# isarandi/metrabs

Measured on AMD Instinct MI355X. Metric: crops/sec (256px, 72 depth bins) at 1/2/4/8 MI355X; MPJPE vs ref, higher is better.
Workload: dtype f32

## Files before the change

metrabs_amd/build.py:

```python
import hashlib
import os
import shutil
import subprocess
import sys
from concurrent.futures import ThreadPoolExecutor

CSRC = os.path.join(os.path.dirname(os.path.abspath(__file__)), 'csrc')
LIB_PATH = os.path.join(CSRC, 'libmetrabs_hip.so')
BUILD_DIR = os.path.join(CSRC, 'build')
ARCH = 'gfx950'
FLAGS = ['-O3', '-std=c++17', '-fPIC', f'--offload-arch={ARCH}', '-Wall', '-Wno-unused-function',
         '-Wno-inline-asm']
EXTRA_FLAGS = {'head_rt.hip': ['-mllvm', '-amdgpu-mfma-vgpr-form=1'],
               'depthwise5x5.hip': ['-fno-slp-vectorize']}


def sources():
    return sorted(f for f in os.listdir(CSRC) if f.endswith('.hip'))


def _hipcc():
    exe = shutil.which('hipcc') or '/opt/rocm/bin/hipcc'
    if not os.path.exists(exe):
        raise RuntimeError('hipcc not found; metrabs_amd needs ROCm to build its HIP kernels')
    return exe


def _digest(path):
    h = hashlib.sha256()
    h.update(' '.join(FLAGS + EXTRA_FLAGS.get(os.path.basename(path), [])).encode())
    for dep in [path] + [os.path.join(CSRC, f) for f in sorted(os.listdir(CSRC)) if f.endswith('.h')] \
            + [os.path.join(os.path.dirname(os.path.dirname(CSRC)), 'include', 'metrabs_hip.h')]:
        with open(dep, 'rb') as f:
            h.update(f.read())
    return h.hexdigest()


def _compile(src, force):
    path = os.path.join(CSRC, src)
    obj = os.path.join(BUILD_DIR, src + '.o')
    stamp = obj + '.sha256'
    digest = _digest(path)
    if not force and os.path.exists(obj) and os.path.exists(stamp) and open(stamp).read() == digest:
        return obj, False
    cmd = [_hipcc(), *FLAGS, *EXTRA_FLAGS.get(src, []), '-c', path, '-o', obj]
    r = subprocess.run(cmd, capture_output=True, text=True)
    if r.returncode != 0:
        raise RuntimeError(f'hipcc failed for {src}:\n{r.stdout}\n{r.stderr}')
    if r.stderr.strip():
        sys.stderr.write(r.stderr)
    with open(stamp, 'w') as f:
        f.write(digest)
    return obj, True


def build_library(force=False, verbose=True):
    os.makedirs(BUILD_DIR, exist_ok=True)
    srcs = sources()
    with ThreadPoolExecutor(max_workers=min(8, len(srcs))) as ex:
        results = list(ex.map(lambda s: _compile(s, force), srcs))
    objs = [o for o, _ in results]
    rebuilt = any(r for _, r in results)
    if rebuilt or force or not os.path.exists(LIB_PATH):
        cmd = [_hipcc(), '-shared', '-fPIC', f'--offload-arch={ARCH}', *objs, '-o', LIB_PATH]
        r = subprocess.run(cmd, capture_output=True, text=True)
        if r.returncode != 0:
            raise RuntimeError(f'link failed:\n{r.stdout}\n{r.stderr}')
        if verbose:
            print(f'built {LIB_PATH} from {len(srcs)} sources')
    elif verbose:
        print(f'{LIB_PATH} is up to date')
    return LIB_PATH


def kernel_resources(src):
    import re
    import tempfile
    path = os.path.join(CSRC, src)
    with tempfile.TemporaryDirectory() as tmp:
        asm = os.path.join(tmp, src + '.s')
        cmd = [_hipcc(), *[f for f in FLAGS if f != '-fPIC'], *EXTRA_FLAGS.get(src, []), '-S',
               '--cuda-device-only', path, '-o', asm]
        r = subprocess.run(cmd, capture_output=True, text=True)
        if r.returncode != 0:
            raise RuntimeError(f'hipcc -S failed for {src}:\n{r.stderr}')
        text = open(asm).read()
    loops = mfma_loop_lane_traffic(text)
    out = []
    meta = text[text.index('amdhsa.kernels:'):] if 'amdhsa.kernels:' in text else ''
    for blk in re.split(r'\n  - ', meta)[1:]:
        if '.vgpr_count:' not in blk:
            continue
        get = lambda k: int(re.search(rf'\.{k}:\s+(\d+)', blk).group(1))
        name = re.search(r'\.name:\s+(\S+)', blk).group(1)
        out.append(dict(name=name, mfma_loops=loops.get(name, []),
                        **{k: get(k) for k in ('vgpr_count', 'agpr_count', 'vgpr_spill_count',
                                               'sgpr_spill_count', 'private_segment_fixed_size',
                                               'group_segment_fixed_size')}))
    return out


def mfma_loop_lane_traffic(asm_text):
    import re
    out = {}
    for m in re.finditer(r'^(_Z\w+):[^\n]*\n', asm_text, flags=re.M):
        name = m.group(1)
        end = asm_text.find('.Lfunc_end', m.end())
        if end < 0:
            continue
        body = asm_text[m.end():end].split('\n')
        labels = {}
        for i, line in enumerate(body):
            lm = re.match(r'^(\.LBB\d+_\d+):', line)
            if lm:
                labels[lm.group(1)] = i
        spans = []
        for i, line in enumerate(body):
            bm = re.search(r's_c?branch\S*\s+(\.LBB\d+_\d+)', line)
            if bm and labels.get(bm.group(1), 1 << 30) <= i:
                spans.append((labels[bm.group(1)], i))
        inner = [sp for sp in spans if not any(o != sp and sp[0] <= o[0] and o[1] <= sp[1] for o in spans)]
        loops = []
        for a, b in inner:
            seg = body[a:b + 1]
            n = lambda key: sum(key in x for x in seg)
            if n('v_mfma'):
                loops.append(dict(mfma=n('v_mfma'), lane_moves=n('v_readlane') + n('v_writelane'),
                                  barriers=n('s_barrier'), dma=n('global_load_lds')))
        out[name] = loops
    return out


if __name__ == '__main__':
    build_library(force='--force' in sys.argv)
```

metrabs_amd/csrc/conv1x1.hip:

```cpp
#include <type_traits>

#include "common.h"

namespace mtr {

typedef float f32x16 __attribute__((ext_vector_type(16)));

constexpr int kC1PadX = 32;
constexpr int kC1PadW = 4;

template <int WM, int WN, int FM, int FN, int BK, int ACT, int PRE>
__global__ __launch_bounds__(64 * WM * WN) void conv1x1_kernel(
    const float* __restrict__ x, const float* __restrict__ w, const float* __restrict__ bias,
    const float* __restrict__ in_bias, const float* __restrict__ gate, const float* __restrict__ residual,
    float* __restrict__ y, int M, int K, int HW, int n_total, FastDiv by_hw) {
  constexpr int NT = 64 * WM * WN;
  constexpr int BM = 32 * FM * WM, BN = 32 * FN * WN;
  constexpr int LDX = BN + kC1PadX, LDW = BM + kC1PadW;
  constexpr int XROW4 = BN / 4;
  constexpr int XPASS = NT / XROW4;
  constexpr int XV = (BK + XPASS - 1) / XPASS;
  constexpr int WPASS = NT / (BK / 4);
  constexpr int WV = (BM + WPASS - 1) / WPASS;
  static_assert(NT % XROW4 == 0 && NT % (BK / 4) == 0, "loader mapping");
  __shared__ float xs[2][BK * LDX];
  __shared__ float ws[2][BK * LDW];

  const int tid = threadIdx.x, lane = tid & 63, wave = tid >> 6;
  const int wm = wave % WM, wn = wave / WM;
  const int m0 = blockIdx.y * BM, n0 = blockIdx.x * BN;
  const long long khw = (long long)K * HW;

  const int xn4 = tid % XROW4, xk0 = tid / XROW4;
  const int xcol = n0 + xn4 * 4;
  const bool xcol_ok = xcol < n_total;
  const unsigned xb = xcol_ok ? fastdiv((unsigned)xcol, by_hw) : 0u;
  const float* xsrc = x + (long long)xb * khw + (xcol - (int)xb * HW);
  const float* gsrc = gate ? gate + (long long)xb * K : nullptr;
  const int wk4 = tid % (BK / 4), wr0 = tid / (BK / 4);

  float4 xr[XV], wr[WV];
  auto load_tile = [&](int k0) {
#pragma unroll
    for (int v = 0; v < XV; ++v) {
      const int k = k0 + xk0 + v * XPASS;
      float4 t = make_float4(0.0f, 0.0f, 0.0f, 0.0f);
      if (xcol_ok && k < K && xk0 + v * XPASS < BK) {
        t = *reinterpret_cast<const float4*>(xsrc + (long long)k * HW);
        if constexpr (PRE >= 0) {
          const float bi = in_bias[k];
          t.x = settled(activate<PRE>(t.x + bi)); t.y = settled(activate<PRE>(t.y + bi));
          t.z = settled(activate<PRE>(t.z + bi)); t.w = settled(activate<PRE>(t.w + bi));
        }
        if (gsrc) {
          const float g = gsrc[k];
          t.x *= g; t.y *= g; t.z *= g; t.w *= g;
        }
      }
      xr[v] = t;
    }
#pragma unroll
    for (int v = 0; v < WV; ++v) {
      const int m = m0 + wr0 + v * WPASS, k = k0 + wk4 * 4;
      float4 t = make_float4(0.0f, 0.0f, 0.0f, 0.0f);
      if (m < M && k < K && wr0 + v * WPASS < BM) t = *reinterpret_cast<const float4*>(w + (long long)m * K + k);
      wr[v] = t;
    }
  };
  auto store_tile = [&](int buf) {
#pragma unroll
    for (int v = 0; v < XV; ++v) {
      const int r = xk0 + v * XPASS;
      if (r < BK) *reinterpret_cast<float4*>(&xs[buf][r * LDX + xn4 * 4]) = xr[v];
    }
#pragma unroll
    for (int v = 0; v < WV; ++v) {
      const int r = wr0 + v * WPASS;
      if (r < BM) {
        float* d = &ws[buf][(wk4 * 4) * LDW + r];
        d[0] = wr[v].x; d[LDW] = wr[v].y; d[2 * LDW] = wr[v].z; d[3 * LDW] = wr[v].w;
      }
    }
  };

  f32x16 acc[FM][FN];
#pragma unroll
  for (int i = 0; i < FM; ++i)
#pragma unroll
    for (int j = 0; j < FN; ++j)
#pragma unroll
      for (int r = 0; r < 16; ++r) acc[i][j][r] = 0.0f;

  const int half = lane >> 5, l32 = lane & 31;
  const int n_tiles = (K + BK - 1) / BK;
  load_tile(0);
  store_tile(0);
  __syncthreads();
  for (int t = 0; t < n_tiles; ++t) {
    const int buf = t & 1;
    if (t + 1 < n_tiles) load_tile((t + 1) * BK);
    const float* xb_ = &xs[buf][half * LDX + wn * (32 * FN) + l32];
    const float* wb_ = &ws[buf][half * LDW + wm * (32 * FM) + l32];
#pragma unroll
    for (int kk = 0; kk < BK; kk += 2) {
      float a[FN], b[FM];
#pragma unroll
      for (int j = 0; j < FN; ++j) a[j] = xb_[kk * LDX + j * 32];
#pragma unroll
      for (int i = 0; i < FM; ++i) b[i] = wb_[kk * LDW + i * 32];
#pragma unroll
      for (int i = 0; i < FM; ++i)
#pragma unroll
        for (int j = 0; j < FN; ++j) acc[i][j] = __builtin_amdgcn_mfma_f32_32x32x2f32(a[j], b[i], acc[i][j], 0, 0, 0);
    }
    if (t + 1 < n_tiles) store_tile(buf ^ 1);
    __syncthreads();
  }

#pragma unroll
  for (int i = 0; i < FM; ++i) {
    const int m = m0 + wm * (32 * FM) + i * 32 + l32;
    if (m >= M) continue;
    const float bm = bias[m];
#pragma unroll
    for (int j = 0; j < FN; ++j) {
#pragma unroll
      for (int g = 0; g < 4; ++g) {
        const int col = n0 + wn * (32 * FN) + j * 32 + 8 * g + 4 * half;
        if (col >= n_total) continue;
        const unsigned b = fastdiv((unsigned)col, by_hw);
        const long long off = ((long long)b * M + m) * HW + (col - (int)b * HW);
        float4 r;
        r.x = activate<ACT>(acc[i][j][4 * g + 0] + bm);
        r.y = activate<ACT>(acc[i][j][4 * g + 1] + bm);
        r.z = activate<ACT>(acc[i][j][4 * g + 2] + bm);
        r.w = activate<ACT>(acc[i][j][4 * g + 3] + bm);
        if (residual) {
          const float4 q = *reinterpret_cast<const float4*>(residual + off);
          r.x += q.x; r.y += q.y; r.z += q.z; r.w += q.w;
        }
        *reinterpret_cast<float4*>(y + off) = r;
      }
    }
  }
}

constexpr int kDkBK = 32, kDkBN = 16, kDkStages = 3;
constexpr int kDkLDW = kDkBK + 4;

typedef float f32x4 __attribute__((ext_vector_type(4)));

constexpr size_t deepk_lds_bytes(int waves) {
  return (size_t)kDkStages * (kDkBK * kDkBN + 32 * waves * kDkLDW) * sizeof(float);
}

template <int WAVES, int ACT, int PRE>
__global__ __launch_bounds__(64 * WAVES) void conv1x1_deepk_kernel(
    const float* __restrict__ x, const float* __restrict__ w, const float* __restrict__ bias,
    const float* __restrict__ in_bias, const float* __restrict__ gate, const float* __restrict__ residual,
    float* __restrict__ y, int M, int K, int HW, int n_total, FastDiv by_hw) {
  constexpr int NT = 64 * WAVES, BM = 32 * WAVES;
  constexpr int XS = kDkBK * kDkBN, WS = BM * kDkLDW;
  static_assert(BM * (kDkBK / 4) == 4 * NT, "W loader mapping");
  extern __shared__ float4 dk_lds[];
  float* xs = reinterpret_cast<float*>(dk_lds);
  float* ws = xs + kDkStages * XS;

  const int tid = threadIdx.x, lane = tid & 63, wave = tid >> 6;
  const int m0 = blockIdx.y * BM, n0 = blockIdx.x * kDkBN;
  const long long khw = (long long)K * HW;

  constexpr int XV = XS / NT;
  static_assert(XV * NT == XS && (XV == 1 || XV == 2), "x loader mapping");
  const int xp = (tid % (kDkBN / XV)) * XV, xk = tid / (kDkBN / XV);
  const int xcol = n0 + xp;
  const bool xcol_ok = xcol < n_total;
  const unsigned xb = xcol_ok ? fastdiv((unsigned)xcol, by_hw) : 0u;
  const float* xsrc = xcol_ok ? x + (long long)xb * khw + (xcol - (int)xb * HW) : x;
  const bool has_gate = gate != nullptr;
  const float* gsrc = has_gate ? gate + (long long)xb * K : x;
  const int wk4 = tid & 7, wr0 = tid >> 3;

  const float4 zero = make_float4(0.0f, 0.0f, 0.0f, 0.0f);
  float4 rw[2][4] = {{zero, zero, zero, zero}, {zero, zero, zero, zero}};
  float rx[2][XV] = {}, rg[2] = {1.0f, 1.0f}, rbi[2] = {0.0f, 0.0f};
  auto load_tile = [&](int kt, auto set) {
    constexpr int P = decltype(set)::value;
    const int k0 = kt * kDkBK;
    const int kx = min(k0 + xk, K - 1);
    if constexpr (XV == 2) {
      const float2 t = *reinterpret_cast<const float2*>(xsrc + (long long)kx * HW);
      rx[P][0] = t.x; rx[P][XV - 1] = t.y;
    } else {
      rx[P][0] = xsrc[(long long)kx * HW];
    }
    rg[P] = gsrc[kx];
    if constexpr (PRE >= 0) rbi[P] = in_bias[kx];
    const int k = min(k0 + wk4 * 4, K - 4);
#pragma unroll
    for (int v = 0; v < 4; ++v) {
      const int m = min(m0 + wr0 + v * (NT / 8), M - 1);
      rw[P][v] = *reinterpret_cast<const float4*>(w + (long long)m * K + k);
    }
  };
  auto store_tile = [&](int stage, int kt, auto set) {
    constexpr int P = decltype(set)::value;
    const int k0 = kt * kDkBK;
    const float g = has_gate ? rg[P] : 1.0f;
    const bool x_ok = xcol_ok && k0 + xk < K;
    float* xd = &xs[stage * XS + xk * kDkBN + xp];
    float v0 = rx[P][0], v1 = rx[P][XV - 1];
    if constexpr (PRE >= 0) {
      v0 = settled(activate<PRE>(v0 + rbi[P]));
      if constexpr (XV == 2) v1 = settled(activate<PRE>(v1 + rbi[P]));
    }
    if constexpr (XV == 2) {
      *reinterpret_cast<float2*>(xd) = make_float2(x_ok ? v0 * g : 0.0f, x_ok ? v1 * g : 0.0f);
    } else {
      *xd = x_ok ? v0 * g : 0.0f;
    }
    const bool k_ok = k0 + wk4 * 4 < K;
#pragma unroll
    for (int v = 0; v < 4; ++v) {
      const int row = wr0 + v * (NT / 8);
      const bool ok = k_ok && m0 + row < M;
      float4 u = rw[P][v];
      u.x = ok ? u.x : 0.0f; u.y = ok ? u.y : 0.0f; u.z = ok ? u.z : 0.0f; u.w = ok ? u.w : 0.0f;
      *reinterpret_cast<float4*>(&ws[stage * WS + row * kDkLDW + wk4 * 4]) = u;
    }
  };

  f32x4 acc[2];
#pragma unroll
  for (int f = 0; f < 2; ++f)
#pragma unroll
    for (int r = 0; r < 4; ++r) acc[f][r] = 0.0f;

  const int c = lane & 15, kg = lane >> 4;
  auto multiply = [&](int stage, int kk0) {
    const float* xb_ = &xs[stage * XS + kg * kDkBN + c];
    const float* wb_ = &ws[stage * WS + (wave * 32 + c) * kDkLDW + kg];
#pragma unroll
    for (int kk = kk0; kk < kk0 + kDkBK / 2; kk += 4) {
      const float a = xb_[kk * kDkBN];
      const float b0 = wb_[kk], b1 = wb_[16 * kDkLDW + kk];
      acc[0] = __builtin_amdgcn_mfma_f32_16x16x4f32(a, b0, acc[0], 0, 0, 0);
      acc[1] = __builtin_amdgcn_mfma_f32_16x16x4f32(a, b1, acc[1], 0, 0, 0);
    }
  };

  const int n_tiles = (K + kDkBK - 1) / kDkBK;
  constexpr std::integral_constant<int, 0> ra{};
  constexpr std::integral_constant<int, 1> rb{};
  load_tile(0, ra);
  if (n_tiles > 1) load_tile(1, rb);
  store_tile(0, 0, ra);
  if (n_tiles > 1) store_tile(1, 1, rb);
  if (n_tiles > 2) load_tile(2, ra);
  __syncthreads();
  int stage = 0;
  auto step = [&](int t, auto hold, auto issue, auto guarded) {
    constexpr bool G = decltype(guarded)::value;
    if (!G || t + 3 < n_tiles) load_tile(t + 3, issue);
    multiply(stage, 0);
    __builtin_amdgcn_sched_barrier(0);
    if (!G || t + 2 < n_tiles) store_tile(stage == 0 ? 2 : stage - 1, t + 2, hold);
    __builtin_amdgcn_sched_barrier(0);
    multiply(stage, kDkBK / 2);
    stage = stage == 2 ? 0 : stage + 1;
    __syncthreads();
  };
  int t = 0;
  for (; t + 4 < n_tiles; t += 2) {
    step(t, ra, rb, std::false_type{});
    step(t + 1, rb, ra, std::false_type{});
  }
  for (; t < n_tiles; t += 2) {
    step(t, ra, rb, std::true_type{});
    if (t + 1 < n_tiles) step(t + 1, rb, ra, std::true_type{});
  }

  const int col = n0 + 4 * kg;
  if (col >= n_total) return;
  const unsigned b = fastdiv((unsigned)col, by_hw);
#pragma unroll
  for (int f = 0; f < 2; ++f) {
    const int m = m0 + wave * 32 + f * 16 + c;
    if (m >= M) continue;
    const float bm = bias[m];
    const long long off = ((long long)b * M + m) * HW + (col - (int)b * HW);
    float4 r;
    r.x = activate<ACT>(acc[f][0] + bm);
    r.y = activate<ACT>(acc[f][1] + bm);
    r.z = activate<ACT>(acc[f][2] + bm);
    r.w = activate<ACT>(acc[f][3] + bm);
    if (residual) {
      const float4 q = *reinterpret_cast<const float4*>(residual + off);
      r.x += q.x; r.y += q.y; r.z += q.z; r.w += q.w;
    }
    *reinterpret_cast<float4*>(y + off) = r;
  }
}

constexpr int kD6BM = 64, kD6BN = 64, kD6BK = 32, kD6Stages = 3, kD6Waves = 8;
constexpr int kD6LDW = kD6BK + 2;

template <int ACT, int PRE>
__global__ __launch_bounds__(64 * kD6Waves) void conv1x1_deep64_kernel(
    const float* __restrict__ x, const float* __restrict__ w, const float* __restrict__ bias,
    const float* __restrict__ in_bias, const float* __restrict__ gate, const float* __restrict__ residual,
    float* __restrict__ y, int M, int K, int HW, int n_total, FastDiv by_hw) {
  constexpr int NT = 64 * kD6Waves, BM = kD6BM, BN = kD6BN, BK = kD6BK, LDW = kD6LDW;
  constexpr int XS = BK * BN, WS = BM * LDW;
  static_assert(BK * (BN / 4) == NT && BM * (BK / 4) == NT, "loader mappings: one 16-byte group of x and of W each");
  __shared__ __attribute__((aligned(16))) float d6_lds[kD6Stages * (XS + WS)];
  float* xs = d6_lds;
  float* ws = d6_lds + kD6Stages * XS;

  const int tid = threadIdx.x, lane = tid & 63, wave = tid >> 6;
  const int wm = wave & 1, wn = wave >> 1;
  const int m0 = blockIdx.y * BM, n0 = blockIdx.x * BN;
  const long long khw = (long long)K * HW;

  const int xn4 = tid & 15, xk = tid >> 4;
  const int xcol = n0 + 4 * xn4;
  const bool xcol_ok = xcol < n_total;
  const unsigned xb = xcol_ok ? fastdiv((unsigned)xcol, by_hw) : 0u;
  const float* xsrc = xcol_ok ? x + (long long)xb * khw + (xcol - (int)xb * HW) : x;
  const bool has_gate = gate != nullptr;
  const float* gsrc = has_gate ? gate + (long long)xb * K : x;
  const int xdst = xk * BN + ((4 * xn4) ^ ((xk & 1) << 4));
  const int wk4 = tid & 7, wr = tid >> 3;
  const float* wsrc = w + (long long)min(m0 + wr, M - 1) * K;
  const bool wrow_ok = m0 + wr < M;
  const int wdst = wr * LDW + 4 * wk4;
  const float* xcur = xsrc + (long long)(3 * BK + xk) * HW;
  const float* gcur = gsrc + 3 * BK + xk;
  const float* bcur = PRE >= 0 ? in_bias + 3 * BK + xk : nullptr;
  const float* wcur = wsrc + 3 * BK + 4 * wk4;
  const long long xadv = (long long)BK * HW;

  const float4 zero = make_float4(0.0f, 0.0f, 0.0f, 0.0f);
  float4 rx[2] = {zero, zero}, rw[2] = {zero, zero};
  float rg[2] = {1.0f, 1.0f}, rbi[2] = {0.0f, 0.0f};
  auto load_tile = [&](int kt, auto set) {
    constexpr int P = decltype(set)::value;
    const int k0 = kt * BK;
    const int kx = min(k0 + xk, K - 1);
    rx[P] = *reinterpret_cast<const float4*>(xsrc + (long long)kx * HW);
    rg[P] = gsrc[kx];
    if constexpr (PRE >= 0) rbi[P] = in_bias[kx];
    rw[P] = *reinterpret_cast<const float4*>(wsrc + min(k0 + 4 * wk4, K - 4));
  };
  auto load_next_whole_tile = [&](auto set) {
    constexpr int P = decltype(set)::value;
    rx[P] = *reinterpret_cast<const float4*>(xcur);
    rg[P] = *gcur;
    if constexpr (PRE >= 0) rbi[P] = *bcur;
    rw[P] = *reinterpret_cast<const float4*>(wcur);
    xcur += xadv; gcur += BK; wcur += BK;
    if constexpr (PRE >= 0) bcur += BK;
  };
  auto store_tile = [&](int stage, int kt, auto set) {
    constexpr int P = decltype(set)::value;
    const int k0 = kt * BK;
    const float g = has_gate ? rg[P] : 1.0f;
    const bool x_ok = xcol_ok && k0 + xk < K;
    float4 v = rx[P];
    if constexpr (PRE >= 0) {
      const float bi = rbi[P];
      v.x = settled(activate<PRE>(v.x + bi)); v.y = settled(activate<PRE>(v.y + bi));
      v.z = settled(activate<PRE>(v.z + bi)); v.w = settled(activate<PRE>(v.w + bi));
    }
    v.x = x_ok ? v.x * g : 0.0f; v.y = x_ok ? v.y * g : 0.0f; v.z = x_ok ? v.z * g : 0.0f; v.w = x_ok ? v.w * g : 0.0f;
    *reinterpret_cast<float4*>(&xs[stage * XS + xdst]) = v;
    const bool ok = wrow_ok && k0 + 4 * wk4 < K;
    const float4 u = rw[P];
    float* wd = &ws[stage * WS + wdst];
    *reinterpret_cast<float2*>(wd) = make_float2(ok ? u.x : 0.0f, ok ? u.y : 0.0f);
    *reinterpret_cast<float2*>(wd + 2) = make_float2(ok ? u.z : 0.0f, ok ? u.w : 0.0f);
  };

  f32x4 acc[2];
#pragma unroll
  for (int f = 0; f < 2; ++f)
#pragma unroll
    for (int r = 0; r < 4; ++r) acc[f][r] = 0.0f;

  const int c = lane & 15, kg = lane >> 4;
  const int xfrag = kg * BN + ((wn * 16 + c) ^ ((kg & 1) << 4));
  const int wfrag = (wm * 32 + c) * LDW + kg;
  auto multiply = [&](int stage, int kk0) {
    const float* xb_ = &xs[stage * XS + xfrag];
    const float* wb_ = &ws[stage * WS + wfrag];
#pragma unroll
    for (int kk = kk0; kk < kk0 + BK / 2; kk += 4) {
      const float a = xb_[kk * BN];
      const float b0 = wb_[kk], b1 = wb_[16 * LDW + kk];
      acc[0] = __builtin_amdgcn_mfma_f32_16x16x4f32(a, b0, acc[0], 0, 0, 0);
      acc[1] = __builtin_amdgcn_mfma_f32_16x16x4f32(a, b1, acc[1], 0, 0, 0);
    }
  };

  const int n_tiles = (K + BK - 1) / BK, n_whole = K / BK;
  constexpr std::integral_constant<int, 0> ra{};
  constexpr std::integral_constant<int, 1> rb{};
  load_tile(0, ra);
  if (n_tiles > 1) load_tile(1, rb);
  store_tile(0, 0, ra);
  if (n_tiles > 1) store_tile(1, 1, rb);
  if (n_tiles > 2) load_tile(2, ra);
  __syncthreads();
  int stage = 0;
  auto step = [&](int t, auto hold, auto issue, auto guarded) {
    constexpr bool G = decltype(guarded)::value;
    if constexpr (!G) load_next_whole_tile(issue);
    else if (t + 3 < n_tiles) load_tile(t + 3, issue);
    multiply(stage, 0);
    __builtin_amdgcn_sched_barrier(0);
    if (!G || t + 2 < n_tiles) store_tile(stage == 0 ? 2 : stage - 1, t + 2, hold);
    __builtin_amdgcn_sched_barrier(0);
    multiply(stage, BK / 2);
    stage = stage == 2 ? 0 : stage + 1;
    __syncthreads();
  };
  int t = 0;
  for (; t + 4 < n_whole; t += 2) {
    step(t, ra, rb, std::false_type{});
    step(t + 1, rb, ra, std::false_type{});
  }
  for (; t < n_tiles; t += 2) {
    step(t, ra, rb, std::true_type{});
    if (t + 1 < n_tiles) step(t + 1, rb, ra, std::true_type{});
  }

  const int col = n0 + wn * 16 + 4 * kg;
  if (col >= n_total) return;
  const unsigned b = fastdiv((unsigned)col, by_hw);
#pragma unroll
  for (int f = 0; f < 2; ++f) {
    const int m = m0 + wm * 32 + f * 16 + c;
    if (m >= M) continue;
    const float bm = bias[m];
    const long long off = ((long long)b * M + m) * HW + (col - (int)b * HW);
    float4 r;
    r.x = activate<ACT>(acc[f][0] + bm);
    r.y = activate<ACT>(acc[f][1] + bm);
    r.z = activate<ACT>(acc[f][2] + bm);
    r.w = activate<ACT>(acc[f][3] + bm);
    if (residual) {
      const float4 q = *reinterpret_cast<const float4*>(residual + off);
      r.x += q.x; r.y += q.y; r.z += q.z; r.w += q.w;
    }
    *reinterpret_cast<float4*>(y + off) = r;
  }
}

constexpr int kStR = 16;
constexpr int kStWaves = 4;
constexpr size_t kStMaxWeight = 64 * 1024;

inline int stream_kpad(int K) { return (K + 2 * kStR - 1) / (2 * kStR) * (2 * kStR); }
inline bool stream_fits(int M, int K) {
  return M <= 96 && (size_t)stream_kpad(K) * ((M + 31) / 32 * 32) * sizeof(float) <= kStMaxWeight;
}

template <int MT, int PRE, bool GATE>
__global__ __launch_bounds__(64 * kStWaves) void conv1x1_stream_kernel(
    const float* __restrict__ x, const float* __restrict__ w, const float* __restrict__ bias,
    const float* __restrict__ in_bias, const float* __restrict__ gate, const float* __restrict__ residual,
    float* __restrict__ y, int M, int K, int HW, int n_total, FastDiv by_hw, int act, int tiles) {
  constexpr int NT = 64 * kStWaves, LDW = 32 * MT;
  extern __shared__ float4 st_lds[];
  const int Kpad = (K + 2 * kStR - 1) / (2 * kStR) * (2 * kStR);
  float* ws = reinterpret_cast<float*>(st_lds);
  float* bs = ws + Kpad * LDW;

  const int tid = threadIdx.x, lane = tid & 63, wave = tid >> 6;
  const int half = lane >> 5, l32 = lane & 31;
  const long long khw = (long long)K * HW;
  const int n_chunks = Kpad / (2 * kStR);
  const int n0 = blockIdx.x * (32 * kStWaves * tiles);

  int col0 = 0;
  bool ok = false;
  const float* xsrc = x;
  const float* gsrc = x;
  auto enter_tile = [&](int tile) {
    col0 = n0 + tile * 32;
    const int col = col0 + l32;
    ok = col < n_total;
    const unsigned b = ok ? fastdiv((unsigned)col, by_hw) : 0u;
    xsrc = x + (long long)b * khw + (long long)half * HW + (ok ? col - (int)b * HW : 0);
    if constexpr (GATE) gsrc = gate + (long long)b * K + half;
  };

  float xa[kStR], xb[kStR], ga[kStR], gb[kStR];
  auto load_chunk = [&](int c, float (&xr)[kStR], float (&gr)[kStR]) {
#pragma unroll
    for (int j = 0; j < kStR; ++j) {
      const int kk = min(c * (2 * kStR) + 2 * j, K - 2);
      xr[j] = xsrc[(long long)kk * HW];
      if constexpr (GATE) gr[j] = gsrc[kk];
    }
  };

  f32x16 acc[MT];
  auto multiply_chunk = [&](int c, const float (&xr)[kStR], const float (&gr)[kStR]) {
#pragma unroll
    for (int j = 0; j < kStR; ++j) {
      const int k = c * (2 * kStR) + 2 * j;
      float v = xr[j];
      if constexpr (PRE >= 0) v = settled(activate<PRE>(v + bs[k + half]));
      if constexpr (GATE) v *= gr[j];
      v = (ok && k < K) ? v : 0.0f;
      const float* wb_ = &ws[(k + half) * LDW + l32];
#pragma unroll
      for (int i = 0; i < MT; ++i) acc[i] = __builtin_amdgcn_mfma_f32_32x32x2f32(v, wb_[i * 32], acc[i], 0, 0, 0);
    }
  };

  enter_tile(wave);
  load_chunk(0, xa, ga);

  for (int e = tid; e < (Kpad / 4) * LDW; e += NT) {
    const int m = e % LDW, k = (e / LDW) * 4;
    float4 t = make_float4(0.0f, 0.0f, 0.0f, 0.0f);
    if (m < M && k < K) t = *reinterpret_cast<const float4*>(w + (long long)m * K + k);
    float* d = &ws[k * LDW + m];
    d[0] = t.x; d[LDW] = t.y; d[2 * LDW] = t.z; d[3 * LDW] = t.w;
  }
  if constexpr (PRE >= 0)
    for (int k = tid; k < Kpad; k += NT) bs[k] = k < K ? in_bias[k] : 0.0f;
  __syncthreads();

  for (int tile = wave;;) {
#pragma unroll
    for (int i = 0; i < MT; ++i)
#pragma unroll
      for (int r = 0; r < 16; ++r) acc[i][r] = 0.0f;
    int c = 0;
    for (; c + 1 < n_chunks; c += 2) {
      load_chunk(c + 1, xb, gb);
      multiply_chunk(c, xa, ga);
      load_chunk(c + 2, xa, ga);
      multiply_chunk(c + 1, xb, gb);
    }
    if (c < n_chunks) multiply_chunk(c, xa, ga);

    auto epilogue = [&](auto act_c) {
      constexpr int ACT = decltype(act_c)::value;
#pragma unroll
      for (int i = 0; i < MT; ++i) {
        const int m = i * 32 + l32;
        if (m >= M) continue;
        const float bm = bias[m];
#pragma unroll
        for (int g = 0; g < 4; ++g) {
          const int col = col0 + 8 * g + 4 * half;
          if (col >= n_total) continue;
          const unsigned b = fastdiv((unsigned)col, by_hw);
          const long long off = ((long long)b * M + m) * HW + (col - (int)b * HW);
          float4 r;
          r.x = activate<ACT>(acc[i][4 * g + 0] + bm);
          r.y = activate<ACT>(acc[i][4 * g + 1] + bm);
          r.z = activate<ACT>(acc[i][4 * g + 2] + bm);
          r.w = activate<ACT>(acc[i][4 * g + 3] + bm);
          if (residual) {
            const float4 q = *reinterpret_cast<const float4*>(residual + off);
            r.x += q.x; r.y += q.y; r.z += q.z; r.w += q.w;
          }
          *reinterpret_cast<float4*>(y + off) = r;
        }
      }
    };
    switch (act) {
      case kActRelu: epilogue(std::integral_constant<int, kActRelu>{}); break;
      case kActSilu: epilogue(std::integral_constant<int, kActSilu>{}); break;
      case kActHardswish: epilogue(std::integral_constant<int, kActHardswish>{}); break;
      default: epilogue(std::integral_constant<int, kActNone>{}); break;
    }

    tile += kStWaves;
    if (tile >= kStWaves * tiles) break;
    enter_tile(tile);
    load_chunk(0, xa, ga);
  }
}

enum Conv1x1Config {
  kCfgWide = 0, kCfgSquare = 1, kCfgTall = 2, kCfgDeepK = 3, kCfgStream = 4, kCfgDeep64 = 5, kCfgCount = 6
};

struct Conv1x1Plan { int cfg, waves_m, bm, bn; };

inline Conv1x1Plan plan_tall(int M) {
  const int w = M <= 160 ? (M + 31) / 32 : 4;
  return {kCfgTall, w, 32 * w, 32};
}
inline Conv1x1Plan plan_deepk(int M) {
  const int w = M <= 128 ? 4 : 8;
  return {kCfgDeepK, w, 32 * w, kDkBN};
}

inline Conv1x1Plan plan_deep64() { return {kCfgDeep64, 2, kD6BM, kD6BN}; }

inline Conv1x1Plan plan_stream(int M, int K, int HW, long long B) {
  if (!stream_fits(M, K)) return plan_tall(M);
  const int t = (B * HW + 127) / 128 >= 2048 ? 2 : 1;
  return {kCfgStream, (M + 31) / 32, (M + 31) / 32 * 32, 32 * kStWaves * t};
}

inline bool deep64_measured_faster(int M, int K, int HW) {
  static const int classes[][3] = {
      {256, 64, 1024}, {128, 256, 256}, {512, 128, 256}, {128, 512, 256},
      {160, 768, 256}, {960, 160, 256}, {160, 960, 256},
      {256, 960, 64},  {1536, 256, 64}, {256, 1536, 64}, {1280, 256, 64},
  };
  for (const auto& c : classes)
    if (c[0] == M && c[1] == K && c[2] == HW) return true;
  return false;
}

inline Conv1x1Plan pick_config(int M, int K, int HW, long long B) {
  const long long n_total = B * HW;
  const long long n_tiles128 = (n_total + 127) / 128;
  if (deep64_measured_faster(M, K, HW)) return plan_deep64();
  if (M == 48 && K <= 192 && HW == 4096 && stream_fits(M, K)) return plan_stream(M, K, HW, B);
  if (M <= 160) return plan_tall(M);
  if (M == 256 && K >= 512) return HW <= 64 ? plan_deepk(M) : plan_tall(M);
  if (M >= 1024 && M % 128 == 0 && K <= 256 && n_tiles128 <= 32) return plan_tall(M);
  if (M % 192 == 0 && (M / 192) * n_tiles128 >= 512) return {kCfgWide, 2, 192, 128};
  return {kCfgSquare, 2, 128, 128};
}

inline int plan_for(int M, int K, int HW, long long B, int config, Conv1x1Plan* p) {
  switch (config) {
    case -1: *p = pick_config(M, K, HW, B); return MTR_OK;
    case kCfgWide: *p = {kCfgWide, 2, 192, 128}; return MTR_OK;
    case kCfgSquare: *p = {kCfgSquare, 2, 128, 128}; return MTR_OK;
    case kCfgTall: *p = plan_tall(M); return MTR_OK;
    case kCfgDeepK: *p = plan_deepk(M); return MTR_OK;
    case kCfgStream: *p = plan_stream(M, K, HW, B); return MTR_OK;
    case kCfgDeep64: *p = plan_deep64(); return MTR_OK;
    default: return MTR_E_PARAM;
  }
}

template <int WM, int WN, int FM, int FN, int BK, int PRE>
static int launch_conv1x1_pre(const float* x, const float* w, const float* bias, const float* in_bias,
                              const float* gate, const float* residual, float* y, int act, int M, int K, int HW,
                              long long n_total, hipStream_t stream) {
  constexpr int BM = 32 * FM * WM, BN = 32 * FN * WN;
  const long long gx = (n_total + BN - 1) / BN, gy = (M + BM - 1) / BM;
  if (gx > 0x7fffffffLL || gy > 65535) return MTR_E_SHAPE;
  const dim3 grid((unsigned)gx, (unsigned)gy), block(64 * WM * WN);
  const FastDiv by_hw = make_fastdiv((unsigned)HW);
  MTR_CLEAR_STALE();
#define MTR_C1_LAUNCH(ACT)                                                                                      \
  hipLaunchKernelGGL((conv1x1_kernel<WM, WN, FM, FN, BK, ACT, PRE>), grid, block, 0, stream, x, w, bias, in_bias, \
                     gate, residual, y, M, K, HW, (int)n_total, by_hw)
  switch (act) {
    case kActNone: MTR_C1_LAUNCH(kActNone); break;
    case kActRelu: MTR_C1_LAUNCH(kActRelu); break;
    case kActSilu: MTR_C1_LAUNCH(kActSilu); break;
    case kActHardswish: MTR_C1_LAUNCH(kActHardswish); break;
    default: return MTR_E_PARAM;
  }
#undef MTR_C1_LAUNCH
  MTR_CHECK_LAUNCH();
  return MTR_OK;
}

template <int WM, int WN, int FM, int FN, int BK>
static int launch_conv1x1_cfg(const float* x, const float* w, const float* bias, const float* in_bias, int in_act,
                              const float* gate, const float* residual, float* y, int act, int M, int K, int HW,
                              long long n_total, hipStream_t stream) {
#define MTR_C1_PRE(PRE) \
  launch_conv1x1_pre<WM, WN, FM, FN, BK, PRE>(x, w, bias, in_bias, gate, residual, y, act, M, K, HW, n_total, stream)
  switch (in_bias ? in_act : -1) {
    case -1: return MTR_C1_PRE(-1);
    case kActNone: return MTR_C1_PRE(kActNone);
    case kActRelu: return MTR_C1_PRE(kActRelu);
    case kActSilu: return MTR_C1_PRE(kActSilu);
    case kActHardswish: return MTR_C1_PRE(kActHardswish);
    default: return MTR_E_PARAM;
  }
#undef MTR_C1_PRE
}

template <int WAVES, int PRE>
static int launch_conv1x1_deepk_pre(const float* x, const float* w, const float* bias, const float* in_bias,
                                    const float* gate, const float* residual, float* y, int act, int M, int K,
                                    int HW, long long n_total, hipStream_t stream) {
  constexpr int BM = 32 * WAVES;
  constexpr size_t lds = deepk_lds_bytes(WAVES);
  const long long gx = (n_total + kDkBN - 1) / kDkBN, gy = (M + BM - 1) / BM;
  if (gx > 0x7fffffffLL || gy > 65535) return MTR_E_SHAPE;
  const dim3 grid((unsigned)gx, (unsigned)gy), block(64 * WAVES);
  const FastDiv by_hw = make_fastdiv((unsigned)HW);
#define MTR_DK_LAUNCH(ACT)                                                                                 \
  do {                                                                                                     \
    if (lds > 64 * 1024) {                                                                                 \
      const int e = allow_dynamic_lds((const void*)conv1x1_deepk_kernel<WAVES, ACT, PRE>, lds);            \
      if (e != MTR_OK) return e;                                                                           \
    }                                                                                                      \
    MTR_CLEAR_STALE();                                                                                     \
    hipLaunchKernelGGL((conv1x1_deepk_kernel<WAVES, ACT, PRE>), grid, block, lds, stream, x, w, bias,      \
                       in_bias, gate, residual, y, M, K, HW, (int)n_total, by_hw);                         \
  } while (0)
  switch (act) {
    case kActNone: MTR_DK_LAUNCH(kActNone); break;
    case kActRelu: MTR_DK_LAUNCH(kActRelu); break;
    case kActSilu: MTR_DK_LAUNCH(kActSilu); break;
    case kActHardswish: MTR_DK_LAUNCH(kActHardswish); break;
    default: return MTR_E_PARAM;
  }
#undef MTR_DK_LAUNCH
  MTR_CHECK_LAUNCH();
  return MTR_OK;
}

template <int WAVES>
static int launch_conv1x1_deepk(const float* x, const float* w, const float* bias, const float* in_bias,
                                int in_act, const float* gate, const float* residual, float* y, int act, int M,
                                int K, int HW, long long n_total, hipStream_t stream) {
#define MTR_DK_PRE(PRE) \
  launch_conv1x1_deepk_pre<WAVES, PRE>(x, w, bias, in_bias, gate, residual, y, act, M, K, HW, n_total, stream)
  switch (in_bias ? in_act : -1) {
    case -1: return MTR_DK_PRE(-1);
    case kActNone: return MTR_DK_PRE(kActNone);
    case kActRelu: return MTR_DK_PRE(kActRelu);
    case kActSilu: return MTR_DK_PRE(kActSilu);
    case kActHardswish: return MTR_DK_PRE(kActHardswish);
    default: return MTR_E_PARAM;
  }
#undef MTR_DK_PRE
}

template <int PRE>
static int launch_conv1x1_deep64_pre(const float* x, const float* w, const float* bias, const float* in_bias,
                                     const float* gate, const float* residual, float* y, int act, int M, int K,
                                     int HW, long long n_total, hipStream_t stream) {
  const long long gx = (n_total + kD6BN - 1) / kD6BN, gy = (M + kD6BM - 1) / kD6BM;
  if (gx > 0x7fffffffLL || gy > 65535) return MTR_E_SHAPE;
  const dim3 grid((unsigned)gx, (unsigned)gy), block(64 * kD6Waves);
  const FastDiv by_hw = make_fastdiv((unsigned)HW);
  MTR_CLEAR_STALE();
#define MTR_D6_LAUNCH(ACT)                                                                                    \
  hipLaunchKernelGGL((conv1x1_deep64_kernel<ACT, PRE>), grid, block, 0, stream, x, w, bias, in_bias, gate,    \
                     residual, y, M, K, HW, (int)n_total, by_hw)
  switch (act) {
    case kActNone: MTR_D6_LAUNCH(kActNone); break;
    case kActRelu: MTR_D6_LAUNCH(kActRelu); break;
    case kActSilu: MTR_D6_LAUNCH(kActSilu); break;
    case kActHardswish: MTR_D6_LAUNCH(kActHardswish); break;
    default: return MTR_E_PARAM;
  }
#undef MTR_D6_LAUNCH
  MTR_CHECK_LAUNCH();
  return MTR_OK;
}

static int launch_conv1x1_deep64(const float* x, const float* w, const float* bias, const float* in_bias,
                                 int in_act, const float* gate, const float* residual, float* y, int act, int M,
                                 int K, int HW, long long n_total, hipStream_t stream) {
#define MTR_D6_PRE(PRE) \
  launch_conv1x1_deep64_pre<PRE>(x, w, bias, in_bias, gate, residual, y, act, M, K, HW, n_total, stream)
  switch (in_bias ? in_act : -1) {
    case -1: return MTR_D6_PRE(-1);
    case kActNone: return MTR_D6_PRE(kActNone);
    case kActRelu: return MTR_D6_PRE(kActRelu);
    case kActSilu: return MTR_D6_PRE(kActSilu);
    case kActHardswish: return MTR_D6_PRE(kActHardswish);
    default: return MTR_E_PARAM;
  }
#undef MTR_D6_PRE
}

template <int MT, int PRE>
static int launch_conv1x1_stream_pre(const float* x, const float* w, const float* bias, const float* in_bias,
                                     const float* gate, const float* residual, float* y, int act, int M, int K,
                                     int HW, long long n_total, int bn, hipStream_t stream) {
  const int kpad = stream_kpad(K);
  const size_t lds = ((size_t)kpad * 32 * MT + (PRE >= 0 ? kpad : 0)) * sizeof(float);
  const long long gx = (n_total + bn - 1) / bn;
  if (gx > 0x7fffffffLL) return MTR_E_SHAPE;
  if (act < kActNone || act > kActHardswish) return MTR_E_PARAM;
  const dim3 grid((unsigned)gx), block(64 * kStWaves);
  const FastDiv by_hw = make_fastdiv((unsigned)HW);
#define MTR_ST_LAUNCH(GATE)                                                                               \
  do {                                                                                                    \
    if (lds > 64 * 1024) {                                                                                \
      const int e = allow_dynamic_lds((const void*)conv1x1_stream_kernel<MT, PRE, GATE>, lds);            \
      if (e != MTR_OK) return e;                                                                          \
    }                                                                                                     \
    MTR_CLEAR_STALE();                                                                                    \
    hipLaunchKernelGGL((conv1x1_stream_kernel<MT, PRE, GATE>), grid, block, lds, stream, x, w, bias,      \
                       in_bias, gate, residual, y, M, K, HW, (int)n_total, by_hw, act,                    \
                       bn / (32 * kStWaves));                                                             \
  } while (0)
  if (gate) MTR_ST_LAUNCH(true); else MTR_ST_LAUNCH(false);
#undef MTR_ST_LAUNCH
  MTR_CHECK_LAUNCH();
  return MTR_OK;
}

template <int MT>
static int launch_conv1x1_stream(const float* x, const float* w, const float* bias, const float* in_bias,
                                 int in_act, const float* gate, const float* residual, float* y, int act, int M,
                                 int K, int HW, long long n_total, int bn, hipStream_t stream) {
#define MTR_ST_PRE(PRE) \
  launch_conv1x1_stream_pre<MT, PRE>(x, w, bias, in_bias, gate, residual, y, act, M, K, HW, n_total, bn, stream)
  switch (in_bias ? in_act : -1) {
    case -1: return MTR_ST_PRE(-1);
    case kActNone: return MTR_ST_PRE(kActNone);
    case kActRelu: return MTR_ST_PRE(kActRelu);
    case kActSilu: return MTR_ST_PRE(kActSilu);
    case kActHardswish: return MTR_ST_PRE(kActHardswish);
    default: return MTR_E_PARAM;
  }
#undef MTR_ST_PRE
}

}

extern "C" int mtr_conv1x1_plan(int M, int K, int HW, long long B, int config, int* plan) {
  if (!plan) return MTR_E_NULL;
  if (B < 0 || M <= 0 || K <= 0 || HW <= 0) return MTR_E_SHAPE;
  mtr::Conv1x1Plan p;
  const int e = mtr::plan_for(M, K, HW, B, config, &p);
  if (e != MTR_OK) return e;
  plan[0] = p.cfg; plan[1] = p.waves_m; plan[2] = p.bm; plan[3] = p.bn;
  return MTR_OK;
}

extern "C" int mtr_conv1x1_bias_act(const void* x, int dtype, const float* weight, const float* bias,
                                    const float* gate, const void* residual, int act, long long B, int M,
                                    int K, int HW, void* y, mtr_stream_t stream) {
  return mtr_conv1x1_bias_act_pre(x, dtype, weight, bias, nullptr, mtr::kActNone, gate, residual, act, B, M, K, HW, y,
                                  stream, -1);
}

extern "C" int mtr_conv1x1_bias_act_opts(const void* x, int dtype, const float* weight, const float* bias,
                                         const float* gate, const void* residual, int act, long long B,
                                         int M, int K, int HW, void* y, mtr_stream_t stream, int config) {
  if (config > mtr::kCfgDeepK) return x && weight && bias && y ? MTR_E_PARAM : MTR_E_NULL;
  return mtr_conv1x1_bias_act_pre(x, dtype, weight, bias, nullptr, mtr::kActNone, gate, residual, act, B, M, K, HW, y,
                                  stream, config);
}

extern "C" int mtr_conv1x1_bias_act_pre(const void* x, int dtype, const float* weight, const float* bias,
                                        const float* in_bias, int in_act, const float* gate, const void* residual,
                                        int act, long long B, int M, int K, int HW, void* y, mtr_stream_t stream,
                                        int config) {
  if (!x || !weight || !bias || !y) return MTR_E_NULL;
  if (dtype != MTR_F32) return MTR_E_DTYPE;
  if (B < 0 || M <= 0 || K <= 0 || HW <= 0) return MTR_E_SHAPE;
  if (HW % 4 || K % 4) return MTR_E_SHAPE;
  if (B * HW > 0x7fffffffLL || (long long)K * HW > 0x7fffffffLL || (long long)M * HW > 0x7fffffffLL)
    return MTR_E_SHAPE;
  if (act < mtr::kActNone || act > mtr::kActHardswish) return MTR_E_PARAM;
  if (in_act < mtr::kActNone || in_act > mtr::kActHardswish) return MTR_E_PARAM;
  if (!in_bias && in_act != mtr::kActNone) return MTR_E_PARAM;
  if (((uintptr_t)x % 16) || ((uintptr_t)weight % 16) || ((uintptr_t)y % 16) || ((uintptr_t)residual % 16) ||
      ((uintptr_t)in_bias % 4))
    return MTR_E_ALIGN;
  if (x == y || (residual && residual == x)) return MTR_E_PARAM;
  if (B == 0) return MTR_OK;
  const float* xf = (const float*)x;
  const float* rf = (const float*)residual;
  float* yf = (float*)y;
  const long long n_total = B * HW;
  hipStream_t s = (hipStream_t)stream;
  mtr::Conv1x1Plan p;
  if (mtr::plan_for(M, K, HW, B, config, &p) != MTR_OK) return MTR_E_PARAM;
#define MTR_C1_ARGS xf, weight, bias, in_bias, in_act, gate, rf, yf, act, M, K, HW, n_total, s
#define MTR_C1_ARGS_ST xf, weight, bias, in_bias, in_act, gate, rf, yf, act, M, K, HW, n_total, p.bn, s
  switch (p.cfg) {
    case mtr::kCfgWide: return mtr::launch_conv1x1_cfg<2, 2, 3, 2, 16>(MTR_C1_ARGS);
    case mtr::kCfgSquare: return mtr::launch_conv1x1_cfg<2, 2, 2, 2, 16>(MTR_C1_ARGS);
    case mtr::kCfgStream:
      switch (p.waves_m) {
        case 1: return mtr::launch_conv1x1_stream<1>(MTR_C1_ARGS_ST);
        case 2: return mtr::launch_conv1x1_stream<2>(MTR_C1_ARGS_ST);
        default: return mtr::launch_conv1x1_stream<3>(MTR_C1_ARGS_ST);
      }
    case mtr::kCfgDeep64: return mtr::launch_conv1x1_deep64(MTR_C1_ARGS);
    case mtr::kCfgDeepK:
      switch (p.waves_m) {
        case 4: return mtr::launch_conv1x1_deepk<4>(MTR_C1_ARGS);
        default: return mtr::launch_conv1x1_deepk<8>(MTR_C1_ARGS);
      }
    default:
      switch (p.waves_m) {
        case 1: return mtr::launch_conv1x1_cfg<1, 1, 1, 1, 16>(MTR_C1_ARGS);
        case 2: return mtr::launch_conv1x1_cfg<2, 1, 1, 1, 16>(MTR_C1_ARGS);
        case 3: return mtr::launch_conv1x1_cfg<3, 1, 1, 1, 16>(MTR_C1_ARGS);
        case 4: return mtr::launch_conv1x1_cfg<4, 1, 1, 1, 32>(MTR_C1_ARGS);
        default: return mtr::launch_conv1x1_cfg<5, 1, 1, 1, 16>(MTR_C1_ARGS);
      }
  }
#undef MTR_C1_ARGS
#undef MTR_C1_ARGS_ST
}
```

Measured before the change: 9400.

## Restructure streaming conv1x1: per-wave column tiles, float2 loads, smaller chunks, tight LDS

Reworks the streaming 1x1 conv kernel so each wave owns one 32- or 64-column tile instead of looping over several tiles, and adds an NW=2 variant that loads two adjacent columns per lane with float2 and reuses each LDS weight fetch across two MFMA accumulator sets. The chunk depth drops from 16 to 4 k-pairs to cut register pressure, and a tail-free fast loop uses pointer increments plus sched_barriers to keep loads and MFMAs interleaved. LDS weight stride now pads M to 16 instead of 32*MT, and launch bounds request higher occupancy for small tiles. The build script also reports load/MFMA runs and vmcnt waits for inspection. Risks include launch-config mismatch (bn must be 128 or 256) and fewer columns per block amortising the weight LDS fill.

```diff
diff --git a/metrabs_amd/build.py b/metrabs_amd/build.py
--- a/metrabs_amd/build.py
+++ b/metrabs_amd/build.py
@@ -125,8 +125,17 @@
             seg = body[a:b + 1]
             n = lambda key: sum(key in x for x in seg)
             if n('v_mfma'):
+                runs = []
+                for x in seg:
+                    kind = 'M' if 'v_mfma' in x else 'L' if re.match(r'\s*(global|buffer|flat)_load_', x) else None
+                    if kind and runs and runs[-1][0] == kind:
+                        runs[-1][1] += 1
+                    elif kind:
+                        runs.append([kind, 1])
+                waits = [int(v) for x in seg if 's_waitcnt' in x for v in re.findall(r'vmcnt\((\d+)\)', x)]
                 loops.append(dict(mfma=n('v_mfma'), lane_moves=n('v_readlane') + n('v_writelane'),
-                                  barriers=n('s_barrier'), dma=n('global_load_lds')))
+                                  barriers=n('s_barrier'), dma=n('global_load_lds'),
+                                  load_mfma_runs=runs, vmcnt_waits=waits))
         out[name] = loops
     return out
 
diff --git a/metrabs_amd/csrc/conv1x1.hip b/metrabs_amd/csrc/conv1x1.hip
--- a/metrabs_amd/csrc/conv1x1.hip
+++ b/metrabs_amd/csrc/conv1x1.hip
@@ -457,6 +457,7 @@
 }
 
 constexpr int kStR = 16;
+constexpr int kStC = 4;
 constexpr int kStWaves = 4;
 constexpr size_t kStMaxWeight = 64 * 1024;
 
@@ -464,63 +465,90 @@
 inline bool stream_fits(int M, int K) {
   return M <= 96 && (size_t)stream_kpad(K) * ((M + 31) / 32 * 32) * sizeof(float) <= kStMaxWeight;
 }
-
-template <int MT, int PRE, bool GATE>
-__global__ __launch_bounds__(64 * kStWaves) void conv1x1_stream_kernel(
+inline __host__ __device__ int stream_ldw(int M) { return (M + 15) / 16 * 16; }
+constexpr int kStTailPad = 16;
+
+template <int MT, int PRE, bool GATE, int NW>
+__global__ __launch_bounds__(64 * kStWaves, (MT * NW <= 4 && !GATE) ? 4 : 1) void conv1x1_stream_kernel(
     const float* __restrict__ x, const float* __restrict__ w, const float* __restrict__ bias,
     const float* __restrict__ in_bias, const float* __restrict__ gate, const float* __restrict__ residual,
-    float* __restrict__ y, int M, int K, int HW, int n_total, FastDiv by_hw, int act, int tiles) {
-  constexpr int NT = 64 * kStWaves, LDW = 32 * MT;
+    float* __restrict__ y, int M, int K, int HW, int n_total, FastDiv by_hw, int act) {
+  constexpr int NT = 64 * kStWaves, CK = 2 * kStC;
+  const int LDW = stream_ldw(M);
+  static_assert(NW == 1 || NW == 2, "one 4-byte or one 8-byte load per lane and k-step");
   extern __shared__ float4 st_lds[];
   const int Kpad = (K + 2 * kStR - 1) / (2 * kStR) * (2 * kStR);
   float* ws = reinterpret_cast<float*>(st_lds);
-  float* bs = ws + Kpad * LDW;
+  float* bs = ws + Kpad * LDW + kStTailPad;
 
   const int tid = threadIdx.x, lane = tid & 63, wave = tid >> 6;
   const int half = lane >> 5, l32 = lane & 31;
   const long long khw = (long long)K * HW;
-  const int n_chunks = Kpad / (2 * kStR);
-  const int n0 = blockIdx.x * (32 * kStWaves * tiles);
-
-  int col0 = 0;
-  bool ok = false;
-  const float* xsrc = x;
-  const float* gsrc = x;
-  auto enter_tile = [&](int tile) {
-    col0 = n0 + tile * 32;
-    const int col = col0 + l32;
-    ok = col < n_total;
-    const unsigned b = ok ? fastdiv((unsigned)col, by_hw) : 0u;
-    xsrc = x + (long long)b * khw + (long long)half * HW + (ok ? col - (int)b * HW : 0);
-    if constexpr (GATE) gsrc = gate + (long long)b * K + half;
-  };
-
-  float xa[kStR], xb[kStR], ga[kStR], gb[kStR];
-  auto load_chunk = [&](int c, float (&xr)[kStR], float (&gr)[kStR]) {
-#pragma unroll
-    for (int j = 0; j < kStR; ++j) {
-      const int kk = min(c * (2 * kStR) + 2 * j, K - 2);
-      xr[j] = xsrc[(long long)kk * HW];
+  const int n_chunks = Kpad / CK, n_whole = K / CK;
+
+  const int col0 = (blockIdx.x * kStWaves + wave) * (32 * NW);
+  const int lcol = col0 + NW * l32;
+  const bool ok = lcol < n_total;
+  const unsigned lb = ok ? fastdiv((unsigned)lcol, by_hw) : 0u;
+  const float* xsrc = x + (long long)lb * khw + (long long)half * HW + (ok ? lcol - (int)lb * HW : 0);
+  const float* gsrc = GATE ? gate + (long long)lb * K + half : x;
+  const float* xcur = xsrc + (long long)CK * HW;
+  const float* gcur = gsrc + CK;
+  const long long xadv = (long long)CK * HW;
+
+  float xa[kStC][NW], xb[kStC][NW], ga[kStC], gb[kStC];
+  auto load_at = [&](const float* p, float (&d)[NW]) {
+    if constexpr (NW == 2) {
+      const float2 t = *reinterpret_cast<const float2*>(p);
+      d[0] = t.x; d[1] = t.y;
+    } else {
+      d[0] = *p;
+    }
+  };
+  auto load_chunk = [&](int c, float (&xr)[kStC][NW], float (&gr)[kStC]) {
+#pragma unroll
+    for (int j = 0; j < kStC; ++j) {
+      const int kk = min(c * CK + 2 * j, K - 2);
+      load_at(xsrc + (long long)kk * HW, xr[j]);
       if constexpr (GATE) gr[j] = gsrc[kk];
     }
   };
-
-  f32x16 acc[MT];
-  auto multiply_chunk = [&](int c, const float (&xr)[kStR], const float (&gr)[kStR]) {
-#pragma unroll
-    for (int j = 0; j < kStR; ++j) {
-      const int k = c * (2 * kStR) + 2 * j;
-      float v = xr[j];
-      if constexpr (PRE >= 0) v = settled(activate<PRE>(v + bs[k + half]));
-      if constexpr (GATE) v *= gr[j];
-      v = (ok && k < K) ? v : 0.0f;
+  auto load_next_whole_chunk = [&](float (&xr)[kStC][NW], float (&gr)[kStC]) {
+#pragma unroll
+    for (int j = 0; j < kStC; ++j) {
+      load_at(xcur + (long long)(2 * j) * HW, xr[j]);
+      if constexpr (GATE) gr[j] = gcur[2 * j];
+    }
+    xcur += xadv;
+    if constexpr (GATE) gcur += CK;
+  };
+
+  f32x16 acc[NW][MT];
+  auto multiply_chunk = [&](int c, const float (&xr)[kStC][NW], const float (&gr)[kStC], auto whole) {
+    constexpr bool WHOLE = decltype(whole)::value;
+#pragma unroll
+    for (int j = 0; j < kStC; ++j) {
+      const int k = c * CK + 2 * j;
+      const bool in = WHOLE ? ok : (ok && k < K);
+      float v[NW];
+#pragma unroll
+      for (int s = 0; s < NW; ++s) {
+        v[s] = xr[j][s];
+        if constexpr (PRE >= 0) v[s] = settled(activate<PRE>(v[s] + bs[k + half]));
+        if constexpr (GATE) v[s] *= gr[j];
+        v[s] = in ? v[s] : 0.0f;
+      }
       const float* wb_ = &ws[(k + half) * LDW + l32];
-#pragma unroll
-      for (int i = 0; i < MT; ++i) acc[i] = __builtin_amdgcn_mfma_f32_32x32x2f32(v, wb_[i * 32], acc[i], 0, 0, 0);
-    }
-  };
-
-  enter_tile(wave);
+      float bf[MT];
+#pragma unroll
+      for (int i = 0; i < MT; ++i) bf[i] = wb_[i * 32];
+#pragma unroll
+      for (int s = 0; s < NW; ++s)
+#pragma unroll
+        for (int i = 0; i < MT; ++i) acc[s][i] = __builtin_amdgcn_mfma_f32_32x32x2f32(v[s], bf[i], acc[s][i], 0, 0, 0);
+    }
+  };
+
   load_chunk(0, xa, ga);
 
   for (int e = tid; e < (Kpad / 4) * LDW; e += NT) {
@@ -530,42 +558,62 @@
     float* d = &ws[k * LDW + m];
     d[0] = t.x; d[LDW] = t.y; d[2 * LDW] = t.z; d[3 * LDW] = t.w;
   }
+  if (tid < kStTailPad) ws[Kpad * LDW + tid] = 0.0f;
   if constexpr (PRE >= 0)
     for (int k = tid; k < Kpad; k += NT) bs[k] = k < K ? in_bias[k] : 0.0f;
   __syncthreads();
 
-  for (int tile = wave;;) {
+#pragma unroll
+  for (int s = 0; s < NW; ++s)
 #pragma unroll
     for (int i = 0; i < MT; ++i)
 #pragma unroll
-      for (int r = 0; r < 16; ++r) acc[i][r] = 0.0f;
-    int c = 0;
-    for (; c + 1 < n_chunks; c += 2) {
-      load_chunk(c + 1, xb, gb);
-      multiply_chunk(c, xa, ga);
-      load_chunk(c + 2, xa, ga);
-      multiply_chunk(c + 1, xb, gb);
-    }
-    if (c < n_chunks) multiply_chunk(c, xa, ga);
-
-    auto epilogue = [&](auto act_c) {
-      constexpr int ACT = decltype(act_c)::value;
-#pragma unroll
-      for (int i = 0; i < MT; ++i) {
-        const int m = i * 32 + l32;
-        if (m >= M) continue;
-        const float bm = bias[m];
-#pragma unroll
-        for (int g = 0; g < 4; ++g) {
-          const int col = col0 + 8 * g + 4 * half;
+      for (int r = 0; r < 16; ++r) acc[s][i][r] = 0.0f;
+
+  int c = 0;
+  for (; c + 2 < n_whole; c += 2) {
+    load_next_whole_chunk(xb, gb);
+    __builtin_amdgcn_sched_barrier(0);
+    multiply_chunk(c, xa, ga, std::true_type{});
+    __builtin_amdgcn_sched_barrier(0);
+    load_next_whole_chunk(xa, ga);
+    __builtin_amdgcn_sched_barrier(0);
+    multiply_chunk(c + 1, xb, gb, std::true_type{});
+    __builtin_amdgcn_sched_barrier(0);
+  }
+  for (; c < n_chunks; c += 2) {
+    if (c + 1 < n_chunks) load_chunk(c + 1, xb, gb);
+    __builtin_amdgcn_sched_barrier(0);
+    multiply_chunk(c, xa, ga, std::false_type{});
+    __builtin_amdgcn_sched_barrier(0);
+    if (c + 1 < n_chunks) {
+      if (c + 2 < n_chunks) load_chunk(c + 2, xa, ga);
+      __builtin_amdgcn_sched_barrier(0);
+      multiply_chunk(c + 1, xb, gb, std::false_type{});
+      __builtin_amdgcn_sched_barrier(0);
+    }
+  }
+
+  auto epilogue = [&](auto act_c) {
+    constexpr int ACT = decltype(act_c)::value;
+#pragma unroll
+    for (int i = 0; i < MT; ++i) {
+      const int m = i * 32 + l32;
+      if (m >= M) continue;
+      const float bm = bias[m];
+#pragma unroll
+      for (int g = 0; g < 4; ++g) {
+#pragma unroll
+        for (int v = 0; v < NW; ++v) {
+          const int col = col0 + 8 * NW * g + 4 * NW * half + 4 * v;
           if (col >= n_total) continue;
           const unsigned b = fastdiv((unsigned)col, by_hw);
           const long long off = ((long long)b * M + m) * HW + (col - (int)b * HW);
-          float4 r;
-          r.x = activate<ACT>(acc[i][4 * g + 0] + bm);
-          r.y = activate<ACT>(acc[i][4 * g + 1] + bm);
-          r.z = activate<ACT>(acc[i][4 * g + 2] + bm);
-          r.w = activate<ACT>(acc[i][4 * g + 3] + bm);
+          float e[4];
+#pragma unroll
+          for (int u = 0; u < 4; ++u)
+            e[u] = activate<ACT>(acc[(4 * v + u) % NW][i][4 * g + (4 * v + u) / NW] + bm);
+          float4 r = make_float4(e[0], e[1], e[2], e[3]);
           if (residual) {
             const float4 q = *reinterpret_cast<const float4*>(residual + off);
             r.x += q.x; r.y += q.y; r.z += q.z; r.w += q.w;
@@ -573,18 +621,13 @@
           *reinterpret_cast<float4*>(y + off) = r;
         }
       }
-    };
-    switch (act) {
-      case kActRelu: epilogue(std::integral_constant<int, kActRelu>{}); break;
-      case kActSilu: epilogue(std::integral_constant<int, kActSilu>{}); break;
-      case kActHardswish: epilogue(std::integral_constant<int, kActHardswish>{}); break;
-      default: epilogue(std::integral_constant<int, kActNone>{}); break;
-    }
-
-    tile += kStWaves;
-    if (tile >= kStWaves * tiles) break;
-    enter_tile(tile);
-    load_chunk(0, xa, ga);
+    }
+  };
+  switch (act) {
+    case kActRelu: epilogue(std::integral_constant<int, kActRelu>{}); break;
+    case kActSilu: epilogue(std::integral_constant<int, kActSilu>{}); break;
+    case kActHardswish: epilogue(std::integral_constant<int, kActHardswish>{}); break;
+    default: epilogue(std::integral_constant<int, kActNone>{}); break;
   }
 }
 
@@ -783,24 +826,29 @@
                                      const float* gate, const float* residual, float* y, int act, int M, int K,
                                      int HW, long long n_total, int bn, hipStream_t stream) {
   const int kpad = stream_kpad(K);
-  const size_t lds = ((size_t)kpad * 32 * MT + (PRE >= 0 ? kpad : 0)) * sizeof(float);
+  const size_t lds = ((size_t)kpad * stream_ldw(M) + kStTailPad + (PRE >= 0 ? kpad : 0)) * sizeof(float);
   const long long gx = (n_total + bn - 1) / bn;
   if (gx > 0x7fffffffLL) return MTR_E_SHAPE;
   if (act < kActNone || act > kActHardswish) return MTR_E_PARAM;
   const dim3 grid((unsigned)gx), block(64 * kStWaves);
   const FastDiv by_hw = make_fastdiv((unsigned)HW);
-#define MTR_ST_LAUNCH(GATE)                                                                               \
+#define MTR_ST_LAUNCH(GATE, NW)                                                                           \
   do {                                                                                                    \
     if (lds > 64 * 1024) {                                                                                \
-      const int e = allow_dynamic_lds((const void*)conv1x1_stream_kernel<MT, PRE, GATE>, lds);            \
+      const int e = allow_dynamic_lds((const void*)conv1x1_stream_kernel<MT, PRE, GATE, NW>, lds);        \
       if (e != MTR_OK) return e;                                                                          \
     }                                                                                                     \
     MTR_CLEAR_STALE();                                                                                    \
-    hipLaunchKernelGGL((conv1x1_stream_kernel<MT, PRE, GATE>), grid, block, lds, stream, x, w, bias,      \
-                       in_bias, gate, residual, y, M, K, HW, (int)n_total, by_hw, act,                    \
-                       bn / (32 * kStWaves));                                                             \
+    hipLaunchKernelGGL((conv1x1_stream_kernel<MT, PRE, GATE, NW>), grid, block, lds, stream, x, w, bias,  \
+                       in_bias, gate, residual, y, M, K, HW, (int)n_total, by_hw, act);                   \
   } while (0)
-  if (gate) MTR_ST_LAUNCH(true); else MTR_ST_LAUNCH(false);
+  if (bn == 64 * kStWaves) {
+    if (gate) MTR_ST_LAUNCH(true, 2); else MTR_ST_LAUNCH(false, 2);
+  } else if (bn == 32 * kStWaves) {
+    if (gate) MTR_ST_LAUNCH(true, 1); else MTR_ST_LAUNCH(false, 1);
+  } else {
+    return MTR_E_PARAM;
+  }
 #undef MTR_ST_LAUNCH
   MTR_CHECK_LAUNCH();
   return MTR_OK;
```

Measured after the change: 9487 (median of 6 runs). About the same (+0.9%).
